# barathanaslan/whisper-ipa

Measured on AMD Instinct MI355X. Metric: audio-seconds/sec transcribed (whisper-small, 30s clips), higher is better.
Workload: dtype bf16

## Files before the change

### whisper_ipa_amd/csrc/cross_absorbed.hip

```cpp
#include <cstdlib>
#include <mutex>
#include <type_traits>

#include "attn_stream.h"
#include "wipa_common.h"

int wipa_cross_absorbed_loop_variant() {
    const char* e = getenv("WIPA_ABS_LOOP");
    const int v = e ? atoi(e) : 1;
    return (v >= 0 && v <= 3) ? v : 1;
}

namespace {

constexpr int FT = 32;
constexpr long long XA_RESIDENT_MB_SHARED = 16;
constexpr long long XA_RESIDENT_MB_LONE = -1;
typedef __attribute__((address_space(3))) void* lds_ptr_a;
typedef int v2i32 __attribute__((ext_vector_type(2)));

struct AbsParams {
    const __bf16* qp;
    const __bf16* xa;
    float* part_m;
    float* part_l;
    float* part_o;
    int Tk, n_splits, tiles_per_split, H;
    int resident_groups;
};

constexpr int POLICY_DEFAULT = 0, POLICY_NT = 2;

__device__ __forceinline__ int swz(int row) { return (row & 7) << 1; }

template <int D>
struct AbsCfg {
    static constexpr int NW = 4;
    static constexpr int ROWB = D * 2;
    static constexpr int TILE = FT * ROWB;
    static constexpr int SX = NW * 2 * 64 * 4 * (int)sizeof(float);
    static constexpr int NBUF = (3 * TILE + SX <= 160 * 1024) ? 3 : 2;
    static constexpr int SMEM = NBUF * TILE + SX;
};

template <int D>
__global__ __launch_bounds__(512, 1) void cross_absorbed_kernel(AbsParams p) {
    typedef AbsCfg<D> X;
    constexpr int NW = X::NW, ROWB = X::ROWB, TILE = X::TILE, NBUF = X::NBUF;
    constexpr int NDMA = TILE / 1024 / NW;
    constexpr int KS = D / NW / 32;
    constexpr int CT = D / NW / 16;
    static_assert(D % (32 * NW) == 0 && TILE % (1024 * NW) == 0, "width");
    extern __shared__ __attribute__((aligned(1024))) char smem[];
    float* sx = reinterpret_cast<float*>(smem + NBUF * TILE);
    const int tid = threadIdx.x, lane = tid & 63;
    const int wave = __builtin_amdgcn_readfirstlane(tid >> 6);
    const int l15 = lane & 15, g = lane >> 4;
    const int split = blockIdx.x, b = blockIdx.y;
    const int tile0 = split * p.tiles_per_split;
    const int n_tiles_total = (p.Tk + FT - 1) / FT;
    const int nt = max(0, min(p.tiles_per_split, n_tiles_total - tile0));
    const __bf16* xb = p.xa + (int64_t)b * p.Tk * D;

// ... 511 lines not shown

template <int D>
__global__ __launch_bounds__(64) void cross_absorb_q_kernel(const __bf16* __restrict__ q, int64_t q_rs, const __bf16* __restrict__ wkT,
                                                            __bf16* __restrict__ qp, int B, int H, float scale) {
    constexpr int CT = D / 4 / 16;
    const int lane = threadIdx.x & 63, wave = blockIdx.z;
    const int l15 = lane & 15, g = lane >> 4;
    const int h = blockIdx.x, b0 = blockIdx.y * 16;
    if (h >= H) {
        for (int e = lane; e < 16 * (D / 4); e += 64) {
            const int bb = b0 + e / (D / 4);
            if (bb < B) qp[((int64_t)bb * 16 + h) * D + wave * (D / 4) + e % (D / 4)] = (__bf16)0.f;
        }
        return;
    }
    const int bq = min(b0 + l15, B - 1);
    bf16x8 qa[2];
#pragma unroll
    for (int ks = 0; ks < 2; ++ks) qa[ks] = *reinterpret_cast<const bf16x8*>(q + (int64_t)bq * q_rs + h * 64 + 32 * ks + 8 * g);
    bf16x8 wb[CT][2];
#pragma unroll
    for (int i = 0; i < CT; ++i)
#pragma unroll
        for (int ks = 0; ks < 2; ++ks)
            wb[i][ks] = *reinterpret_cast<const bf16x8*>(wkT + (int64_t)(wave * (D / 4) + 16 * i + l15) * D + h * 64 + 32 * ks + 8 * g);
#pragma unroll
    for (int i = 0; i < CT; ++i) {
        const int c0 = wave * (D / 4) + 16 * i;
        f32x4 acc = f32x4{0.f, 0.f, 0.f, 0.f};
#pragma unroll
        for (int ks = 0; ks < 2; ++ks) acc = __builtin_amdgcn_mfma_f32_16x16x32_bf16(qa[ks], wb[i][ks], acc, 0, 0, 0);
#pragma unroll
        for (int r = 0; r < 4; ++r) {
            const int bb = b0 + 4 * g + r;
            if (bb < B) qp[((int64_t)bb * 16 + h) * D + c0 + l15] = (__bf16)(acc[r] * scale);
        }
    }
}

template <int D>
struct MergeCfg {
#ifndef WIPA_MERGE_KQ
#define WIPA_MERGE_KQ 96
#endif
#ifndef WIPA_MERGE_CL
#define WIPA_MERGE_CL 4
#endif
    static constexpr int KQ = (D % 96 == 0) ? WIPA_MERGE_KQ : (D == 512 ? 64 : 128);
    static constexpr int NWM = D / KQ;
    static constexpr int KS = KQ / 32;
    static constexpr int CL = WIPA_MERGE_CL;
};

template <int D, bool OUTP = false, int NS = 4>
__global__ __launch_bounds__(64 * MergeCfg<D>::NWM) void cross_merge_proj_kernel(
    const float* __restrict__ part_m, const float* __restrict__ part_l, const float* __restrict__ part_o, int n_splits,
    const __bf16* __restrict__ wv, const float* __restrict__ bv, __bf16* __restrict__ out, int64_t o_rs, int B,
    const __bf16* __restrict__ wo = nullptr, const float* __restrict__ bo = nullptr, float* __restrict__ slabs_out = nullptr,
    int64_t slab_stride = 0) {
    constexpr int KQ = MergeCfg<D>::KQ, KS = MergeCfg<D>::KS, NWM = MergeCfg<D>::NWM;
    static_assert(KQ % 32 == 0 && NWM * KQ == D, "width");
    constexpr int CL = MergeCfg<D>::CL;
    constexpr int NTO = D / 16;
    constexpr int NTOW = (NTO + NWM - 1) / NWM;
    __shared__ __attribute__((aligned(16))) float red[NWM][CL][64 + 4];
    __shared__ __attribute__((aligned(16))) __bf16 vh[OUTP ? CL : 1][64 + 8];
    const int tid = threadIdx.x, lane = tid & 63, w = tid >> 6;
    const int l15 = lane & 15, g = lane >> 4;
    const int h = blockIdx.x, b0 = blockIdx.y * CL;
    const int bc = min(b0 + (l15 & (CL - 1)), B - 1);
    bf16x8 wq[4][KS];
#pragma unroll
    for (int nt = 0; nt < 4; ++nt)
#pragma unroll
        for (int ks = 0; ks < KS; ++ks)
            wq[nt][ks] = *reinterpret_cast<const bf16x8*>(wv + (int64_t)(h * 64 + 16 * nt + l15) * D + w * KQ + 32 * ks + 8 * g);
    bf16x8 wof[OUTP ? NTOW : 1][2];
    if constexpr (OUTP) {
#pragma unroll
        for (int i = 0; i < NTOW; ++i) {
            const int nt = min(w * NTOW + i, NTO - 1);
#pragma unroll
            for (int ks = 0; ks < 2; ++ks)
                wof[i][ks] = *reinterpret_cast<const bf16x8*>(wo + (int64_t)(16 * nt + l15) * D + h * 64 + 32 * ks + 8 * g);
        }
    }
    float pm[NS], pl[NS];
#pragma unroll
    for (int s = 0; s < NS; ++s) {
        const int sc = NS == 4 ? min(s, n_splits - 1) : s;
        pm[s] = part_m[((int64_t)bc * n_splits + sc) * 16 + h];
        pl[s] = part_l[((int64_t)bc * n_splits + sc) * 16 + h];
    }
    f32x4 po[KS][NS][2];
#pragma unroll
    for (int ks = 0; ks < KS; ++ks)
#pragma unroll
        for (int s = 0; s < NS; ++s) {
            const int sc = NS == 4 ? min(s, n_splits - 1) : s;
            const float* pr = part_o + (((int64_t)bc * n_splits + sc) * 16 + h) * D + w * KQ + 32 * ks + 8 * g;
            po[ks][s][0] = *reinterpret_cast<const f32x4*>(pr);
            po[ks][s][1] = *reinterpret_cast<const f32x4*>(pr + 4);
        }
    __builtin_amdgcn_sched_barrier(0);
    float ws[NS];
    {
        float M = NEG_BIG;
#pragma unroll
        for (int s = 0; s < NS; ++s)
            if (NS < 4 || s < n_splits) M = fmaxf(M, pm[s]);
        float Lsum = 0.f;
#pragma unroll
        for (int s = 0; s < NS; ++s) {
            ws[s] = (NS < 4 || s < n_splits) ? __expf(pm[s] - M) : 0.f;
            Lsum = __builtin_fmaf(ws[s], pl[s], Lsum);
        }
        const float inv = 1.0f / Lsum;
#pragma unroll
        for (int s = 0; s < NS; ++s) ws[s] *= inv;
    }
    f32x4 acc[4] = {f32x4{0.f, 0.f, 0.f, 0.f}, f32x4{0.f, 0.f, 0.f, 0.f}, f32x4{0.f, 0.f, 0.f, 0.f}, f32x4{0.f, 0.f, 0.f, 0.f}};
#pragma unroll
    for (int ks = 0; ks < KS; ++ks) {
        f32x4 lo = {0.f, 0.f, 0.f, 0.f}, hi = {0.f, 0.f, 0.f, 0.f};
#pragma unroll
        for (int s = 0; s < NS; ++s) {
            const f32x4 w4 = {ws[s], ws[s], ws[s], ws[s]};
            lo = __builtin_elementwise_fma(w4, po[ks][s][0], lo);
            hi = __builtin_elementwise_fma(w4, po[ks][s][1], hi);
        }
        bf16x8 a;
#pragma unroll
        for (int e = 0; e < 4; ++e) {
            a[e] = (__bf16)lo[e];
            a[4 + e] = (__bf16)hi[e];
        }
#pragma unroll
        for (int nt = 0; nt < 4; ++nt) acc[nt] = __builtin_amdgcn_mfma_f32_16x16x32_bf16(a, wq[nt][ks], acc[nt], 0, 0, 0);
    }
    if (4 * g < CL) {
#pragma unroll
        for (int nt = 0; nt < 4; ++nt)
#pragma unroll
            for (int r = 0; r < 4; ++r)
                if (4 * g + r < CL) red[w][4 * g + r][16 * nt + l15] = acc[nt][r];
    }
    __syncthreads();
    for (int e = tid; e < CL * 64; e += 64 * NWM) {
        const int row = e >> 6, j = e & 63;
        float o = 0.f;
#pragma unroll
        for (int v = 0; v < NWM; ++v) o += red[v][row][j];
        const __bf16 val = (__bf16)(o + bv[h * 64 + j]);
        if constexpr (OUTP) vh[row][j] = val;
        else if (b0 + row < B) out[(int64_t)(b0 + row) * o_rs + h * 64 + j] = val;
    }
    if constexpr (OUTP) {
        __syncthreads();
        const bf16x8 a0 = *reinterpret_cast<const bf16x8*>(&vh[l15 & (CL - 1)][8 * g]);
        const bf16x8 a1 = *reinterpret_cast<const bf16x8*>(&vh[l15 & (CL - 1)][32 + 8 * g]);
#pragma unroll
        for (int i = 0; i < NTOW; ++i) {
            const int nt = w * NTOW + i;
            if (nt < NTO) {
                f32x4 acc2 = {0.f, 0.f, 0.f, 0.f};
                acc2 = __builtin_amdgcn_mfma_f32_16x16x32_bf16(a0, wof[i][0], acc2, 0, 0, 0);
                acc2 = __builtin_amdgcn_mfma_f32_16x16x32_bf16(a1, wof[i][1], acc2, 0, 0, 0);
                if (4 * g < CL) {
                    const float bias = (h == 0) ? bo[16 * nt + l15] : 0.f;
#pragma unroll
                    for (int r = 0; r < 4; ++r)
                        if (4 * g + r < CL && b0 + 4 * g + r < B)
                            slabs_out[(int64_t)h * slab_stride + (int64_t)(b0 + 4 * g + r) * D + 16 * nt + l15] = acc2[r] + bias;
                }
            }
        }
    }
}

struct AbsPrologueParams {
    const float* x_in;
    float* x_out;
    const float* slabs;
    const float* ln_w;
    const float* ln_b;
    const __bf16* wq;
    const float* bq;
    const __bf16* wkT;
    __bf16* qp;
    int64_t slab_stride;
    int n_slabs, B, H;
    float eps, q_scale, k_scale;
};

template <int D, int CG>
__global__ __launch_bounds__(512) void cross_absorb_prologue_kernel(AbsPrologueParams p) {
    constexpr int KS = D / 32;
    constexpr int KSW = (KS + 7) / 8;
    constexpr int NT = D / 16;
    constexpr int NTW = (NT + 7) / 8;
    constexpr int LROW = D + 8;
    constexpr int V4 = D / 256;
    static_assert(D % 256 == 0 || D == 384, "width");
    __shared__ __attribute__((aligned(16))) __bf16 lnx[16][LROW];
    __shared__ __attribute__((aligned(16))) float red[8][16][64 + 4];
    __shared__ __attribute__((aligned(16))) __bf16 qh[16][64 + 8];
    const int tid = threadIdx.x, lane = tid & 63;
    const int wave = __builtin_amdgcn_readfirstlane(tid >> 6);
// ... 70 lines not shown
            if (b0 + row < p.B) *reinterpret_cast<bf16x8*>(p.qp + ((int64_t)(b0 + row) * 16 + hp) * D + 8 * c8) = bf16x8{0, 0, 0, 0, 0, 0, 0, 0};
        }
    }
    __syncthreads();
    {
        f32x4 acc[4] = {f32x4{0.f, 0.f, 0.f, 0.f}, f32x4{0.f, 0.f, 0.f, 0.f}, f32x4{0.f, 0.f, 0.f, 0.f}, f32x4{0.f, 0.f, 0.f, 0.f}};
#pragma unroll
        for (int i = 0; i < KSW; ++i) {
            const int ks = wave * KSW + i;
            if (ks < KS) {
                const bf16x8 a = *reinterpret_cast<const bf16x8*>(&lnx[l15][32 * ks + 8 * g]);
#pragma unroll
                for (int nt = 0; nt < 4; ++nt) acc[nt] = __builtin_amdgcn_mfma_f32_16x16x32_bf16(a, wqf[nt][i], acc[nt], 0, 0, 0);
            }
        }
#pragma unroll
        for (int nt = 0; nt < 4; ++nt)
#pragma unroll
            for (int r = 0; r < 4; ++r) red[wave][4 * g + r][16 * nt + l15] = acc[nt][r];
    }
    __syncthreads();
#pragma unroll
    for (int i = 0; i < CG / 8; ++i) {
        const int e = tid + 512 * i, row = e >> 6, j = e & 63;
        float q = 0.f;
#pragma unroll
        for (int w = 0; w < 8; ++w) q += red[w][row][j];
        qh[row][j] = (__bf16)((q + p.bq[h * 64 + j]) * p.q_scale);
    }
    if constexpr (CG < 16) {
        for (int e = tid; e < (16 - CG) * 64; e += 512) qh[CG + (e >> 6)][e & 63] = (__bf16)0.f;
    }
    __syncthreads();
    {
        const bf16x8 a0 = *reinterpret_cast<const bf16x8*>(&qh[l15][8 * g]);
        const bf16x8 a1 = *reinterpret_cast<const bf16x8*>(&qh[l15][32 + 8 * g]);
#pragma unroll
        for (int i = 0; i < NTW; ++i) {
            const int nt = wave * NTW + i;
            if (nt < NT) {
                f32x4 acc = {0.f, 0.f, 0.f, 0.f};
                acc = __builtin_amdgcn_mfma_f32_16x16x32_bf16(a0, wkf[i][0], acc, 0, 0, 0);
                acc = __builtin_amdgcn_mfma_f32_16x16x32_bf16(a1, wkf[i][1], acc, 0, 0, 0);
#pragma unroll
                for (int r = 0; r < 4; ++r) {
                    const int bb_ = b0 + 4 * g + r;
                    if (4 * g + r < CG && bb_ < p.B) p.qp[((int64_t)bb_ * 16 + h) * D + 16 * nt + l15] = (__bf16)(acc[r] * p.k_scale);
                }
            }
        }
    }
}

template <int D, bool OUTP, typename... Args>
void launch_merge(int lv, int S, dim3 grid, hipStream_t s, Args... args) {
    constexpr int T = 64 * MergeCfg<D>::NWM;
    const int ns = (lv == 1 || lv == 3) ? S : 4;
    if (ns == 1) hipLaunchKernelGGL((cross_merge_proj_kernel<D, OUTP, 1>), grid, dim3(T), 0, s, args...);
    else if (ns == 2) hipLaunchKernelGGL((cross_merge_proj_kernel<D, OUTP, 2>), grid, dim3(T), 0, s, args...);
    else if (ns == 3) hipLaunchKernelGGL((cross_merge_proj_kernel<D, OUTP, 3>), grid, dim3(T), 0, s, args...);
    else hipLaunchKernelGGL((cross_merge_proj_kernel<D, OUTP, 4>), grid, dim3(T), 0, s, args...);
}

template <int D>
int launch_attn(int lv, const AbsParams& p_in, int B, hipStream_t s) {
    const char* e = getenv("WIPA_ABS_KERNEL");
    const bool pipe = lv == 1 || lv == 2;
    AbsParams p = p_in;
    p.resident_groups = wipa_cross_absorbed_resident_groups(B, D, p.Tk, p.n_splits);
    if ((e && atoi(e) == 1) || (D > 768 && !(e && atoi(e) == 2)))
        hipLaunchKernelGGL((cross_absorbed_kernel<D>), dim3(p.n_splits, B), dim3(64 * AbsCfg<D>::NW), AbsCfg<D>::SMEM, s, p);
    else if constexpr (D > 768) {
        if (pipe) hipLaunchKernelGGL((cross_absorbed_v2_kernel<D, 2, true>), dim3(p.n_splits, B), dim3(128), (AbsCfg2<D, 2>::SMEM), s, p);
        else hipLaunchKernelGGL((cross_absorbed_v2_kernel<D, 2, false>), dim3(p.n_splits, B), dim3(128), (AbsCfg2<D, 2>::SMEM), s, p);
    } else {
        static const int waves = [] { const char* w = getenv("WIPA_ABS_WAVES"); return w ? atoi(w) : 3; }();
        if (waves == 2 && pipe) hipLaunchKernelGGL((cross_absorbed_v2_kernel<D, 2, true>), dim3(p.n_splits, B), dim3(128), (AbsCfg2<D, 2>::SMEM), s, p);
        else if (waves == 2) hipLaunchKernelGGL((cross_absorbed_v2_kernel<D, 2, false>), dim3(p.n_splits, B), dim3(128), (AbsCfg2<D, 2>::SMEM), s, p);
        else if (pipe) hipLaunchKernelGGL((cross_absorbed_v2_kernel<D, 3, true>), dim3(p.n_splits, B), dim3(192), (AbsCfg2<D, 3>::SMEM), s, p);
        else hipLaunchKernelGGL((cross_absorbed_v2_kernel<D, 3, false>), dim3(p.n_splits, B), dim3(192), (AbsCfg2<D, 3>::SMEM), s, p);
    }
    return WIPA_OK;
}

AbsParams abs_params(void* scratch, int B, int d, int Tk, int S, int H, const void* xa) {
    char* sc = (char*)scratch;
    AbsParams p = {};
    p.qp = (const __bf16*)sc; p.xa = (const __bf16*)xa;
    p.part_m = (float*)(sc + (size_t)B * 16 * d * 2);
    p.part_l = p.part_m + (size_t)B * S * 16;
    p.part_o = p.part_l + (size_t)B * S * 16;
    p.Tk = Tk; p.n_splits = S; p.H = H;
    const int tiles = (Tk + FT - 1) / FT;
    p.tiles_per_split = (tiles + S - 1) / S;
    return p;
}

template <typename F>
int for_width(int d, F f) {
    if (d == 384) return f(std::integral_constant<int, 384>());
    if (d == 512) return f(std::integral_constant<int, 512>());
    if (d == 768) return f(std::integral_constant<int, 768>());
    if (d == 1024) return f(std::integral_constant<int, 1024>());
    return WIPA_ERR_ARG;
}

}

extern "C" int wipa_cross_absorbed_splits(int want, int Tk) {
    const int tiles = (Tk + FT - 1) / FT;
// ... 44 lines not shown
                                        hipFuncAttributeMaxDynamicSharedMemorySize, AbsCfg2<D, 3>::SMEM);
            if (e == hipSuccess)
                e = hipFuncSetAttribute(reinterpret_cast<const void*>(&cross_absorbed_v2_kernel<D, 3, false>),
                                        hipFuncAttributeMaxDynamicSharedMemorySize, AbsCfg2<D, 3>::SMEM);
        }
        if (e == hipSuccess)
            e = hipFuncSetAttribute(reinterpret_cast<const void*>(&cross_absorbed_v2_kernel<D, 2, true>),
                                    hipFuncAttributeMaxDynamicSharedMemorySize, AbsCfg2<D, 2>::SMEM);
        if (e == hipSuccess)
            e = hipFuncSetAttribute(reinterpret_cast<const void*>(&cross_absorbed_v2_kernel<D, 2, false>),
                                    hipFuncAttributeMaxDynamicSharedMemorySize, AbsCfg2<D, 2>::SMEM);
        return WIPA_OK;
    });
    WIPA_CHECK_HIP(e);
    done[wi] = true;
    return WIPA_OK;
}

extern "C" int wipa_cross_absorbed_stream(const void* xa, void* scratch, size_t scratch_bytes, int B, int H, int d, int Tk, int n_splits,
                                          wipa_stream_t stream) {
    WIPA_REQUIRE(xa && scratch && B > 0 && H >= 1 && H <= 16 && d == H * 64 && (d == 384 || d == 512 || d == 768 || d == 1024) && Tk >= 1 &&
                     n_splits >= 0 && n_splits <= 4,
                 "wipa_cross_absorbed_stream: bad arguments");
    WIPA_REQUIRE(scratch_bytes >= wipa_cross_absorbed_scratch_bytes(B, d, Tk), "wipa_cross_absorbed_stream: scratch too small");
    const int rc0 = wipa_cross_absorbed_init(d);
    if (rc0 != WIPA_OK) return rc0;
    const int S = wipa_cross_absorbed_splits(n_splits, Tk);
    const AbsParams p = abs_params(scratch, B, d, Tk, S, H, xa);
    const int rc = for_width(d, [&](auto width) { return launch_attn<decltype(width)::value>(wipa_cross_absorbed_loop_variant(), p, B, (hipStream_t)stream); });
    if (rc != WIPA_OK) return rc;
    WIPA_LAUNCH_CHECK();
    return WIPA_OK;
}

extern "C" int wipa_cross_absorbed_attention(const void* q, int64_t q_row_stride, const void* wkT, const void* xa, const void* wv,
                                             const float* bv, void* out, int64_t out_row_stride, void* scratch, size_t scratch_bytes,
                                             int B, int H, int d, int Tk, float k_scale, int n_splits, wipa_stream_t stream) {
    WIPA_REQUIRE(q && wkT && xa && wv && bv && out && scratch, "wipa_cross_absorbed_attention: null pointer");
    WIPA_REQUIRE(n_splits >= 0 && n_splits <= 4, "wipa_cross_absorbed_attention: n_splits %d (0 = default, 1..4)", n_splits);
    WIPA_REQUIRE(B > 0 && B <= 65535 && H >= 1 && H <= 16 && d == H * 64 && (d == 384 || d == 512 || d == 768 || d == 1024) && Tk >= 1,
                 "wipa_cross_absorbed_attention: bf16, <= 16 heads of 64, d in {384, 512, 768, 1024} (got H=%d d=%d)", H, d);
    WIPA_REQUIRE(q_row_stride % 8 == 0 && out_row_stride >= d && ((uintptr_t)q % 16) == 0 && ((uintptr_t)xa % 16) == 0 &&
                     ((uintptr_t)wkT % 16) == 0 && ((uintptr_t)wv % 16) == 0 && ((uintptr_t)scratch % 16) == 0,
                 "wipa_cross_absorbed_attention: operands must be 16-byte aligned");
    WIPA_REQUIRE((int64_t)Tk * d * 2 < ((int64_t)1 << 31), "wipa_cross_absorbed_attention: clip too long for 32-bit tile offsets");
    WIPA_REQUIRE(scratch_bytes >= wipa_cross_absorbed_scratch_bytes(B, d, Tk), "wipa_cross_absorbed_attention: scratch too small");
    hipStream_t s = (hipStream_t)stream;
    {
        const int rc0 = wipa_cross_absorbed_init(d);
        if (rc0 != WIPA_OK) return rc0;
    }
    const int S = wipa_cross_absorbed_splits(n_splits, Tk);
    const AbsParams p = abs_params(scratch, B, d, Tk, S, H, xa);
    const dim3 gq(16, (B + 15) / 16, 4), gm(H, (B + WIPA_MERGE_CL - 1) / WIPA_MERGE_CL);
    const int lv = wipa_cross_absorbed_loop_variant();
    const char* st_env = getenv("WIPA_ABS_STAGES");
    const int stages = st_env ? atoi(st_env) : 7;
    const int rc = for_width(d, [&](auto width) {
        constexpr int D = decltype(width)::value;
        int rc = WIPA_OK;
        if (stages & 1)
            hipLaunchKernelGGL((cross_absorb_q_kernel<D>), gq, dim3(64), 0, s, (const __bf16*)q, q_row_stride, (const __bf16*)wkT,
                               const_cast<__bf16*>(p.qp), B, H, k_scale);
        if (stages & 2) rc = launch_attn<D>(lv, p, B, s);
        if (rc == WIPA_OK && (stages & 4))
            launch_merge<D, false>(lv, S, gm, s, (const float*)p.part_m, (const float*)p.part_l, (const float*)p.part_o, S, (const __bf16*)wv, bv,
                                   (__bf16*)out, out_row_stride, B, (const __bf16*)nullptr, (const float*)nullptr, (float*)nullptr, (int64_t)0);
        return rc;
    });
    if (rc != WIPA_OK) return rc;
    WIPA_LAUNCH_CHECK();
    return WIPA_OK;
}

static int absorbed_block(const wipa_cross_block_desc* c, const void* wkT, const void* wv, const float* bv, const void* wo, const float* bo,
                          float* slabs_out, int64_t slab_stride, void* scratch, size_t scratch_bytes, wipa_stream_t stream);

extern "C" int wipa_decode_cross_absorbed_block(const wipa_cross_block_desc* c, const void* wkT, const void* wv, const float* bv, void* scratch,
                                                size_t scratch_bytes, wipa_stream_t stream) {
    WIPA_REQUIRE(c && c->out, "wipa_decode_cross_absorbed_block: null pointer");
    return absorbed_block(c, wkT, wv, bv, nullptr, nullptr, nullptr, 0, scratch, scratch_bytes, stream);
}

extern "C" int wipa_decode_cross_absorbed_block_out(const wipa_cross_block_desc* c, const void* wkT, const void* wv, const float* bv,
                                                    const void* wo, const float* bo, float* slabs_out, int64_t slab_stride, void* scratch,
                                                    size_t scratch_bytes, wipa_stream_t stream) {
    WIPA_REQUIRE(c && wo && bo && slabs_out && slab_stride >= (int64_t)c->B * c->d && ((uintptr_t)wo % 16) == 0,
                 "wipa_decode_cross_absorbed_block_out: null pointer / short slab stride");
    return absorbed_block(c, wkT, wv, bv, wo, bo, slabs_out, slab_stride, scratch, scratch_bytes, stream);
}

static int absorbed_block(const wipa_cross_block_desc* c, const void* wkT, const void* wv, const float* bv, const void* wo, const float* bo,
                          float* slabs_out, int64_t slab_stride, void* scratch, size_t scratch_bytes, wipa_stream_t stream) {
    WIPA_REQUIRE(c && c->x_in && c->x_out && c->ln_w && c->ln_b && c->wq && c->bq && c->kv && (c->out || wo) && wkT && wv && bv && scratch,
                 "wipa_decode_cross_absorbed_block: null pointer");
    WIPA_REQUIRE(c->x_in != c->x_out, "wipa_decode_cross_absorbed_block: x_out must not alias x_in");
    const int B = c->B, H = c->H, d = c->d, Tk = c->Tk;
    WIPA_REQUIRE(c->dtype == WIPA_BF16 && B > 0 && B <= 65535 * 16 && H >= 1 && H <= 16 && d == H * 64 &&
                     (d == 384 || d == 512 || d == 768 || d == 1024) && Tk >= 1 && c->n_slabs >= 0 && c->n_slabs <= 4 && !c->bias_o &&
                     c->cross_splits >= 0 && c->cross_splits <= 4,
                 "wipa_decode_cross_absorbed_block: bf16, <= 16 heads of 64, d in {384, 512, 768, 1024}, <= 4 slabs, no separate bias, "
                 "cross_splits 0..4");
    WIPA_REQUIRE(c->n_slabs == 0 || c->slabs, "wipa_decode_cross_absorbed_block: slabs missing");
    WIPA_REQUIRE((int64_t)Tk * d * 2 < ((int64_t)1 << 31), "wipa_decode_cross_absorbed_block: clip too long for 32-bit tile offsets");
    WIPA_REQUIRE(scratch_bytes >= wipa_cross_absorbed_scratch_bytes(B, d, Tk), "wipa_decode_cross_absorbed_block: scratch too small");
    hipStream_t s = (hipStream_t)stream;
    const int S = wipa_cross_absorbed_splits(c->cross_splits, Tk);
    const AbsParams p = abs_params(scratch, B, d, Tk, S, H, c->kv);
    AbsPrologueParams q = {};
    q.x_in = c->x_in; q.x_out = c->x_out; q.slabs = c->slabs; q.ln_w = c->ln_w; q.ln_b = c->ln_b;
    q.wq = (const __bf16*)c->wq; q.bq = c->bq; q.wkT = (const __bf16*)wkT; q.qp = const_cast<__bf16*>(p.qp);
    q.slab_stride = c->slab_stride; q.n_slabs = c->n_slabs; q.B = B; q.H = H;
    q.eps = c->eps; q.q_scale = c->qk_scale; q.k_scale = c->qk_scale;
    const int lv = wipa_cross_absorbed_loop_variant();
    static const int cg = [] { const char* e = getenv("WIPA_ABS_PROLOGUE_CLIPS"); return e ? atoi(e) : 8; }();
    const dim3 gp(H, cg == 8 ? (B + 7) / 8 : (B + 15) / 16), gm(H, (B + WIPA_MERGE_CL - 1) / WIPA_MERGE_CL);
    const int rc = for_width(d, [&](auto width) {
        constexpr int D = decltype(width)::value;
        if (cg == 8) hipLaunchKernelGGL((cross_absorb_prologue_kernel<D, 8>), gp, dim3(512), 0, s, q);
        else hipLaunchKernelGGL((cross_absorb_prologue_kernel<D, 16>), gp, dim3(512), 0, s, q);
        const int rc = launch_attn<D>(lv, p, B, s);
        if (rc == WIPA_OK && wo)
            launch_merge<D, true>(lv, S, gm, s, (const float*)p.part_m, (const float*)p.part_l, (const float*)p.part_o, S, (const __bf16*)wv, bv,
                                  (__bf16*)nullptr, (int64_t)d, B, (const __bf16*)wo, bo, slabs_out, slab_stride);
        else if (rc == WIPA_OK)
            launch_merge<D, false>(lv, S, gm, s, (const float*)p.part_m, (const float*)p.part_l, (const float*)p.part_o, S, (const __bf16*)wv, bv,
                                   (__bf16*)c->out, (int64_t)d, B, (const __bf16*)nullptr, (const float*)nullptr, (float*)nullptr, (int64_t)0);
        return rc;
    });
    if (rc != WIPA_OK) return rc;
    WIPA_LAUNCH_CHECK();
    return WIPA_OK;
}
```

### whisper_ipa_amd/csrc/runtime.hip

```cpp
#include <algorithm>
#include <cstdarg>
#include <cstdlib>
#include <cstring>
#include <strings.h>
#include <map>
#include <mutex>
#include <tuple>
#include <vector>

#include "wipa_common.h"

static thread_local char g_err[512] = "";
void wipa_set_error(const char* fmt, ...) {
    va_list ap;
    va_start(ap, fmt);
    vsnprintf(g_err, sizeof(g_err), fmt, ap);
    va_end(ap);
}
extern "C" const char* wipa_last_error(void) { return g_err; }
extern "C" int wipa_version(void) { return 100; }

extern "C" int wipa_stream_create_cu_limited(int n_cus, wipa_stream_t* out) {
    int dev = 0, total = 0;
    WIPA_CHECK_HIP(hipGetDevice(&dev));
// ... 832 lines not shown
    hipStream_t s = (hipStream_t)stream;
    char* st = (char*)state;
    const DecScratch S = dec_scratch(cfg, B);
    RT_CALL(wipa_decode_fused_init());
    RT_CALL(wipa_gemm_init());
    WIPA_CHECK_HIP(hipMemsetAsync(st + L.tokens, 0, (size_t)B * L.ld_tok * 4, s));
    WIPA_CHECK_HIP(hipMemsetAsync(st + L.pos, 0, 512, s));
    WIPA_CHECK_HIP(hipMemsetAsync(st + L.sum_logprobs, 0, (size_t)B * 4, s));
    WIPA_CHECK_HIP(hipMemsetAsync(st + L.scratch + S.posd, 0, 8, s));
    int t4[4] = {0, 0, 0, 0};
    for (int i = 0; i < n_init; ++i) t4[i] = initial_tokens_host[i];
    hipLaunchKernelGGL(fill_tokens_kernel, dim3((B + 63) / 64), dim3(64), 0, s, (int32_t*)(st + L.tokens), L.ld_tok, B, n_init,
                       t4[0], t4[1], t4[2], t4[3], (const int32_t*)nullptr);
    WIPA_LAUNCH_CHECK();
    return WIPA_OK;
}

extern "C" int wipa_decoder_run(const wipa_model_cfg* cfg, const void* const* w, void* state, size_t state_bytes, int B, int n_init,
                                int eot, const float* mask_first, const float* mask_always, int n_steps, int use_graph,
                                wipa_stream_t stream) {
    return wipa_decoder_run_rules(cfg, w, state, state_bytes, B, n_init, eot, mask_first, mask_always, n_steps, use_graph, nullptr, stream);
}

extern "C" int wipa_decoder_run_rules(const wipa_model_cfg* cfg, const void* const* w, void* state, size_t state_bytes, int B, int n_init,
                                      int eot, const float* mask_first, const float* mask_always, int n_steps, int use_graph,
                                      const wipa_decode_rules* rules, wipa_stream_t stream) {
    RT_CALL(cfg_check(cfg));
    SplitScope split_scope(cfg);
    WIPA_REQUIRE(w && state && mask_first && mask_always && B > 0 && n_steps >= 0, "wipa_decoder_run: bad arguments");
    RT_CALL(rules_servable("wipa_decoder_run_rules", cfg, B, eot, rules));
    RulesScope rules_scope(rules);
    W8Scope w8_scope(cfg, w);
    const wipa_dec_layout L = dec_layout(cfg, B);
    RT_CALL(state_fits("wipa_decoder_run", L, state_bytes));
    char* st = (char*)state;
    hipStream_t s = (hipStream_t)stream;
    RT_CALL(init_before_capture(cfg));
    if (n_steps == 0) return WIPA_OK;
    WIPA_CHECK_HIP(hipMemsetAsync(done_counter_of(st, L), 0, sizeof(int32_t), s));
    if (step_needs_head(cfg, B)) RT_CALL(enqueue_step_head(cfg, w, st, L, B, stream));
    const bool lean_ok = !use_fused_step(cfg, B) && logits_fused(cfg, B);
    struct LeanScope {
        explicit LeanScope(bool v) { t_lean_logits = v; }
        ~LeanScope() { t_lean_logits = false; }
    };
    if (!use_graph || !graphs_allowed()) {
        for (int i = 0; i < n_steps; ++i) {
            LeanScope lean(lean_ok && i + 1 < n_steps);
            RT_CALL(enqueue_decode_step(cfg, w, st, L, B, n_init, eot, mask_first, mask_always, stream));
        }
        return WIPA_OK;
    }
    WIPA_REQUIRE(s != nullptr, "wipa_decoder_run: graph capture needs a non-default stream");
    const int variant = cfg->dtype * 2 + t_f32_split + 4 * decode_mode(cfg, B) + 16 * cfg->dec_w_dtype + 64 * cfg->dec_cross_absorbed * (absorbed_block_fused() ? 2 : 1) + 256 * (int)tail_fused() + 512 * (int)absorbed_merge_out() + 1024 * cfg->dec_cross_splits + 8192 * (int)lean_ok + 16384 * (cfg->dec_cross_absorbed ? wipa_cross_absorbed_loop_variant() : 0);
    auto step_graph = [&](bool lean, hipGraphExec_t* out) -> int {
        hipGraphExec_t exec = nullptr;
        const GraphKey key(state, (const void*)w, (const void*)mask_first, (const void*)mask_always, B, n_init, eot, variant, cfg->weights_generation,
                           lean ? 2 : 0, rules ? rules->timestamp_begin : 0, rules ? rules->no_timestamps : 0,
                           rules ? rules->max_initial_timestamp_index : 0);
        {
            std::lock_guard<std::mutex> lk(g_graph_mu);
            auto it = g_graphs.find(key);
            if (it != g_graphs.end()) exec = it->second;
        }
        if (!exec) {
            hipGraph_t graph = nullptr;
            WIPA_CHECK_HIP(hipStreamBeginCapture(s, hipStreamCaptureModeRelaxed));
            int rc;
            {
                LeanScope scope(lean);
                rc = enqueue_decode_step(cfg, w, st, L, B, n_init, eot, mask_first, mask_always, stream);
            }
            const hipError_t ee = hipStreamEndCapture(s, &graph);
            if (rc != WIPA_OK) {
                if (graph) hipGraphDestroy(graph);
                return rc;
            }
            WIPA_CHECK_HIP(ee);
            WIPA_CHECK_HIP(hipGraphInstantiate(&exec, graph, nullptr, nullptr, 0));
            WIPA_CHECK_HIP(hipGraphDestroy(graph));
            std::lock_guard<std::mutex> lk(g_graph_mu);
            g_graphs[key] = exec;
        }
        *out = exec;
        return WIPA_OK;
    };
    hipGraphExec_t full = nullptr, lean = nullptr;
    RT_CALL(step_graph(false, &full));
    if (lean_ok && n_steps > 1) RT_CALL(step_graph(true, &lean));
    for (int i = 0; i < n_steps; ++i) WIPA_CHECK_HIP(hipGraphLaunch((lean && i + 1 < n_steps) ? lean : full, s));
    return WIPA_OK;
}

extern "C" int wipa_decoder_prefill(const wipa_model_cfg* cfg, const void* const* w, void* state, size_t state_bytes, int B,
                                    int n_init, int eot, const float* mask_first, const float* mask_always, int use_graph,
                                    wipa_stream_t stream) {
    return wipa_decoder_prefill_rules(cfg, w, state, state_bytes, B, n_init, eot, mask_first, mask_always, use_graph, nullptr, stream);
}

extern "C" int wipa_decoder_prefill_rules(const wipa_model_cfg* cfg, const void* const* w, void* state, size_t state_bytes, int B,
                                          int n_init, int eot, const float* mask_first, const float* mask_always, int use_graph,
                                          const wipa_decode_rules* rules, wipa_stream_t stream) {
    RT_CALL(cfg_check(cfg));
    SplitScope split_scope(cfg);
    WIPA_REQUIRE(w && state && mask_first && mask_always && B > 0, "wipa_decoder_prefill: bad arguments");
    RT_CALL(rules_servable("wipa_decoder_prefill_rules", cfg, B, eot, rules));
    RulesScope rules_scope(rules);
    WIPA_REQUIRE(n_init >= 1 && n_init <= MAX_PROMPT, "wipa_decoder_prefill: 1..%d prompt tokens (got %d)", MAX_PROMPT, n_init);
    W8Scope w8_scope(cfg, w);
    const wipa_dec_layout L = dec_layout(cfg, B);
    RT_CALL(state_fits("wipa_decoder_prefill", L, state_bytes));
    char* st = (char*)state;
    auto enqueue = [&]() -> int {
        if (n_init == 1) {
            if (step_needs_head(cfg, B)) RT_CALL(enqueue_step_head(cfg, w, st, L, B, stream));
            return enqueue_decode_step(cfg, w, st, L, B, n_init, eot, mask_first, mask_always, stream);
        }
        return enqueue_prefill(cfg, w, st, L, B, n_init, eot, mask_first, mask_always, stream);
    };
    hipStream_t s = (hipStream_t)stream;
    RT_CALL(init_before_capture(cfg));
    WIPA_CHECK_HIP(hipMemsetAsync(done_counter_of(st, L), 0, sizeof(int32_t), s));
    if (!use_graph || s == nullptr || !graphs_allowed()) return enqueue();
    hipGraphExec_t exec = nullptr;
    const GraphKey key(state, (const void*)w, (const void*)mask_first, (const void*)mask_always, B, n_init, eot, cfg->dtype * 2 + t_f32_split + 4 * decode_mode(cfg, B) + 16 * cfg->dec_w_dtype + 64 * cfg->dec_cross_absorbed * (absorbed_block_fused() ? 2 : 1) + 256 * (int)tail_fused() + 512 * (int)absorbed_merge_out() + 1024 * cfg->dec_cross_splits + 8192 * (int)(!use_fused_step(cfg, B) && logits_fused(cfg, B)) + 16384 * (cfg->dec_cross_absorbed ? wipa_cross_absorbed_loop_variant() : 0), cfg->weights_generation, 1,
                       rules ? rules->timestamp_begin : 0, rules ? rules->no_timestamps : 0, rules ? rules->max_initial_timestamp_index : 0);
    {
        std::lock_guard<std::mutex> lk(g_graph_mu);
        auto it = g_graphs.find(key);
        if (it != g_graphs.end()) exec = it->second;
    }
    if (!exec) {
        hipGraph_t graph = nullptr;
        WIPA_CHECK_HIP(hipStreamBeginCapture(s, hipStreamCaptureModeRelaxed));
        const int rc = enqueue();
        const hipError_t ee = hipStreamEndCapture(s, &graph);
        if (rc != WIPA_OK) {
            if (graph) hipGraphDestroy(graph);
            return rc;
        }
        WIPA_CHECK_HIP(ee);
        WIPA_CHECK_HIP(hipGraphInstantiate(&exec, graph, nullptr, nullptr, 0));
        WIPA_CHECK_HIP(hipGraphDestroy(graph));
        std::lock_guard<std::mutex> lk(g_graph_mu);
        g_graphs[key] = exec;
    }
    WIPA_CHECK_HIP(hipGraphLaunch(exec, s));
    return WIPA_OK;
}

extern "C" int wipa_decoder_release(void* state) {
    std::lock_guard<std::mutex> lk(g_graph_mu);
    for (auto it = g_graphs.begin(); it != g_graphs.end();) {
        if (std::get<0>(it->first) == state) {
            hipGraphExecDestroy(it->second);
            it = g_graphs.erase(it);
        } else {
            ++it;
        }
    }
    return WIPA_OK;
}

namespace {
struct TfWs {
    size_t x, ln, qkv, q, ao, h, ckv, total;
};
TfWs tf_ws(const wipa_model_cfg* c, int B, int T) {
    const size_t e = wipa_dtype_size(c->dtype), d = c->n_text_state, M = (size_t)B * T;
    TfWs w;
    size_t o = 0;
    w.x = o;   o += align256(M * d * 4);
    w.ln = o;  o += align256(M * d * e);
    w.qkv = o; o += align256(M * 3 * d * e);
    w.q = o;   o += align256(M * d * e);
    w.ao = o;  o += align256(M * d * e);
    w.h = o;   o += align256(M * 4 * d * e);
    w.ckv = o; o += align256((size_t)B * 2 * c->n_text_head * c->n_audio_ctx * 64 * e);
// ... 89 lines not shown
```

### whisper_ipa_amd/csrc/wipa_common.h

```cpp
#pragma once
#include <hip/hip_runtime.h>
#include <stdint.h>
#include <stdio.h>

#include "wipa.h"

typedef __attribute__((ext_vector_type(8))) __bf16 bf16x8;
typedef __attribute__((ext_vector_type(4))) __bf16 bf16x4;
typedef __attribute__((ext_vector_type(4))) float f32x4;
typedef __attribute__((ext_vector_type(16))) float f32x16;

#define WIPA_WAVE 64

void wipa_set_error(const char* fmt, ...);
int wipa_decode_fused_init();
int wipa_gemm_init();
int wipa_cross_absorbed_loop_variant();

#define WIPA_CHECK_HIP(expr)                                                        \
    do {                                                                            \
        hipError_t _e = (expr);                                                     \
        if (_e != hipSuccess) {                                                     \
            wipa_set_error("%s:%d %s -> %s", __FILE__, __LINE__, #expr, hipGetErrorString(_e)); \
            return WIPA_ERR_HIP;                                                    \
        }                                                                           \
    } while (0)

#define WIPA_REQUIRE(cond, ...)                \
    do {                                       \
        if (!(cond)) {                         \
            wipa_set_error(__VA_ARGS__);       \
            return WIPA_ERR_ARG;               \
        }                                      \
    } while (0)

#define WIPA_LAUNCH_CHECK()                                                          \
    do {                                                                             \
        hipError_t _e = hipGetLastError();                                           \
        if (_e != hipSuccess) {                                                      \
            wipa_set_error("%s:%d launch -> %s", __FILE__, __LINE__, hipGetErrorString(_e)); \
            return WIPA_ERR_HIP;                                                     \
        }                                                                            \
    } while (0)

static inline size_t wipa_dtype_size(int dt) { return dt == WIPA_BF16 ? 2 : 4; }

#ifdef __HIPCC__
__device__ __forceinline__ float wipa_bf16_to_f32(unsigned short h) {
    return __uint_as_float(((unsigned int)h) << 16);
}

template <typename T>
__device__ __forceinline__ float to_f32(T v);
template <>
__device__ __forceinline__ float to_f32<float>(float v) { return v; }
template <>
__device__ __forceinline__ float to_f32<__bf16>(__bf16 v) { return (float)v; }

template <typename T>
__device__ __forceinline__ T from_f32(float v);
template <>
__device__ __forceinline__ float from_f32<float>(float v) { return v; }
template <>
__device__ __forceinline__ __bf16 from_f32<__bf16>(float v) { return (__bf16)v; }

template <typename T>
struct Vec16;
template <>
struct Vec16<float> {
    static constexpr int EPL = 4;
// ... 93 lines not shown
```

Baseline: 27720.

## Split cross-attention merge projection over output column halves with 8-clip tiles

For D=768 without the fused out-projection, the merge+V-projection kernel gets a new grid shape. It now uses 8 clips per workgroup and splits the head's 64 output columns across two workgroups along z, with each workgroup computing 32 columns. This is used only when the resulting grid has at most 256 workgroups, and it is on by default behind WIPA_STEP_PLACEMENT. The goal is to spread the small decode-step merge across more CUs and cut per-workgroup MFMA and weight-register work. The cost is that each split re-reads the partial attention outputs and recomputes the softmax merge weights.

```diff
diff --git a/whisper_ipa_amd/csrc/cross_absorbed.hip b/whisper_ipa_amd/csrc/cross_absorbed.hip
--- a/whisper_ipa_amd/csrc/cross_absorbed.hip
+++ b/whisper_ipa_amd/csrc/cross_absorbed.hip
@@ -9,6 +9,11 @@
     const char* e = getenv("WIPA_ABS_LOOP");
     const int v = e ? atoi(e) : 1;
     return (v >= 0 && v <= 3) ? v : 1;
+}
+
+int wipa_step_placement() {
+    const char* e = getenv("WIPA_STEP_PLACE");
+    return (e && atoi(e) == 0) ? 0 : 1;
 }
 
 namespace {
@@ -626,7 +631,7 @@
     static constexpr int CL = WIPA_MERGE_CL;
 };
 
-template <int D, bool OUTP = false, int NS = 4>
+template <int D, bool OUTP = false, int NS = 4, int CL = MergeCfg<D>::CL, int CT = 4>
 __global__ __launch_bounds__(64 * MergeCfg<D>::NWM) void cross_merge_proj_kernel(
     const float* __restrict__ part_m, const float* __restrict__ part_l, const float* __restrict__ part_o, int n_splits,
     const __bf16* __restrict__ wv, const float* __restrict__ bv, __bf16* __restrict__ out, int64_t o_rs, int B,
@@ -634,21 +639,22 @@
     int64_t slab_stride = 0) {
     constexpr int KQ = MergeCfg<D>::KQ, KS = MergeCfg<D>::KS, NWM = MergeCfg<D>::NWM;
     static_assert(KQ % 32 == 0 && NWM * KQ == D, "width");
-    constexpr int CL = MergeCfg<D>::CL;
+    static_assert((CT == 4 || !OUTP) && (CT == 1 || CT == 2 || CT == 4), "the out projection needs the head's 64 values in one workgroup");
     constexpr int NTO = D / 16;
     constexpr int NTOW = (NTO + NWM - 1) / NWM;
-    __shared__ __attribute__((aligned(16))) float red[NWM][CL][64 + 4];
+    __shared__ __attribute__((aligned(16))) float red[NWM][CL][16 * CT + 4];
     __shared__ __attribute__((aligned(16))) __bf16 vh[OUTP ? CL : 1][64 + 8];
     const int tid = threadIdx.x, lane = tid & 63, w = tid >> 6;
     const int l15 = lane & 15, g = lane >> 4;
     const int h = blockIdx.x, b0 = blockIdx.y * CL;
+    const int c0 = CT < 4 ? 16 * CT * (int)blockIdx.z : 0;
     const int bc = min(b0 + (l15 & (CL - 1)), B - 1);
-    bf16x8 wq[4][KS];
-#pragma unroll
-    for (int nt = 0; nt < 4; ++nt)
+    bf16x8 wq[CT][KS];
+#pragma unroll
+    for (int nt = 0; nt < CT; ++nt)
 #pragma unroll
         for (int ks = 0; ks < KS; ++ks)
-            wq[nt][ks] = *reinterpret_cast<const bf16x8*>(wv + (int64_t)(h * 64 + 16 * nt + l15) * D + w * KQ + 32 * ks + 8 * g);
+            wq[nt][ks] = *reinterpret_cast<const bf16x8*>(wv + (int64_t)(h * 64 + c0 + 16 * nt + l15) * D + w * KQ + 32 * ks + 8 * g);
     bf16x8 wof[OUTP ? NTOW : 1][2];
     if constexpr (OUTP) {
 #pragma unroll
@@ -693,7 +699,9 @@
 #pragma unroll
         for (int s = 0; s < NS; ++s) ws[s] *= inv;
     }
-    f32x4 acc[4] = {f32x4{0.f, 0.f, 0.f, 0.f}, f32x4{0.f, 0.f, 0.f, 0.f}, f32x4{0.f, 0.f, 0.f, 0.f}, f32x4{0.f, 0.f, 0.f, 0.f}};
+    f32x4 acc[CT];
+#pragma unroll
+    for (int nt = 0; nt < CT; ++nt) acc[nt] = f32x4{0.f, 0.f, 0.f, 0.f};
 #pragma unroll
     for (int ks = 0; ks < KS; ++ks) {
         f32x4 lo = {0.f, 0.f, 0.f, 0.f}, hi = {0.f, 0.f, 0.f, 0.f};
@@ -710,24 +718,24 @@
             a[4 + e] = (__bf16)hi[e];
         }
 #pragma unroll
-        for (int nt = 0; nt < 4; ++nt) acc[nt] = __builtin_amdgcn_mfma_f32_16x16x32_bf16(a, wq[nt][ks], acc[nt], 0, 0, 0);
+        for (int nt = 0; nt < CT; ++nt) acc[nt] = __builtin_amdgcn_mfma_f32_16x16x32_bf16(a, wq[nt][ks], acc[nt], 0, 0, 0);
     }
     if (4 * g < CL) {
 #pragma unroll
-        for (int nt = 0; nt < 4; ++nt)
+        for (int nt = 0; nt < CT; ++nt)
 #pragma unroll
             for (int r = 0; r < 4; ++r)
                 if (4 * g + r < CL) red[w][4 * g + r][16 * nt + l15] = acc[nt][r];
     }
     __syncthreads();
-    for (int e = tid; e < CL * 64; e += 64 * NWM) {
-        const int row = e >> 6, j = e & 63;
+    for (int e = tid; e < CL * 16 * CT; e += 64 * NWM) {
+        const int row = e / (16 * CT), j = e % (16 * CT);
         float o = 0.f;
 #pragma unroll
         for (int v = 0; v < NWM; ++v) o += red[v][row][j];
-        const __bf16 val = (__bf16)(o + bv[h * 64 + j]);
+        const __bf16 val = (__bf16)(o + bv[h * 64 + c0 + j]);
         if constexpr (OUTP) vh[row][j] = val;
-        else if (b0 + row < B) out[(int64_t)(b0 + row) * o_rs + h * 64 + j] = val;
+        else if (b0 + row < B) out[(int64_t)(b0 + row) * o_rs + h * 64 + c0 + j] = val;
     }
     if constexpr (OUTP) {
         __syncthreads();
@@ -904,10 +912,23 @@
     }
 }
 
+constexpr int PLACE_MAX_WORKGROUPS = 256;
+
 template <int D, bool OUTP, typename... Args>
-void launch_merge(int lv, int S, dim3 grid, hipStream_t s, Args... args) {
+void launch_merge(int lv, int S, bool place, int H, int B, hipStream_t s, Args... args) {
     constexpr int T = 64 * MergeCfg<D>::NWM;
     const int ns = (lv == 1 || lv == 3) ? S : 4;
+    if constexpr (D == 768 && !OUTP) {
+        const dim3 g2(H, (B + 7) / 8, 2);
+        if (place && (int64_t)g2.x * g2.y * g2.z <= PLACE_MAX_WORKGROUPS) {
+            if (ns == 1) hipLaunchKernelGGL((cross_merge_proj_kernel<D, false, 1, 8, 2>), g2, dim3(T), 0, s, args...);
+            else if (ns == 2) hipLaunchKernelGGL((cross_merge_proj_kernel<D, false, 2, 8, 2>), g2, dim3(T), 0, s, args...);
+            else if (ns == 3) hipLaunchKernelGGL((cross_merge_proj_kernel<D, false, 3, 8, 2>), g2, dim3(T), 0, s, args...);
+            else hipLaunchKernelGGL((cross_merge_proj_kernel<D, false, 4, 8, 2>), g2, dim3(T), 0, s, args...);
+            return;
+        }
+    }
+    const dim3 grid(H, (B + WIPA_MERGE_CL - 1) / WIPA_MERGE_CL);
     if (ns == 1) hipLaunchKernelGGL((cross_merge_proj_kernel<D, OUTP, 1>), grid, dim3(T), 0, s, args...);
     else if (ns == 2) hipLaunchKernelGGL((cross_merge_proj_kernel<D, OUTP, 2>), grid, dim3(T), 0, s, args...);
     else if (ns == 3) hipLaunchKernelGGL((cross_merge_proj_kernel<D, OUTP, 3>), grid, dim3(T), 0, s, args...);
@@ -1058,8 +1079,9 @@
     }
     const int S = wipa_cross_absorbed_splits(n_splits, Tk);
     const AbsParams p = abs_params(scratch, B, d, Tk, S, H, xa);
-    const dim3 gq(16, (B + 15) / 16, 4), gm(H, (B + WIPA_MERGE_CL - 1) / WIPA_MERGE_CL);
+    const dim3 gq(16, (B + 15) / 16, 4);
     const int lv = wipa_cross_absorbed_loop_variant();
+    const bool place_merge = wipa_step_placement() != 0;
     const char* st_env = getenv("WIPA_ABS_STAGES");
     const int stages = st_env ? atoi(st_env) : 7;
     const int rc = for_width(d, [&](auto width) {
@@ -1070,7 +1092,7 @@
                                const_cast<__bf16*>(p.qp), B, H, k_scale);
         if (stages & 2) rc = launch_attn<D>(lv, p, B, s);
         if (rc == WIPA_OK && (stages & 4))
-            launch_merge<D, false>(lv, S, gm, s, (const float*)p.part_m, (const float*)p.part_l, (const float*)p.part_o, S, (const __bf16*)wv, bv,
+            launch_merge<D, false>(lv, S, place_merge, H, B, s, (const float*)p.part_m, (const float*)p.part_l, (const float*)p.part_o, S, (const __bf16*)wv, bv,
                                    (__bf16*)out, out_row_stride, B, (const __bf16*)nullptr, (const float*)nullptr, (float*)nullptr, (int64_t)0);
         return rc;
     });
@@ -1120,17 +1142,18 @@
     q.eps = c->eps; q.q_scale = c->qk_scale; q.k_scale = c->qk_scale;
     const int lv = wipa_cross_absorbed_loop_variant();
     static const int cg = [] { const char* e = getenv("WIPA_ABS_PROLOGUE_CLIPS"); return e ? atoi(e) : 8; }();
-    const dim3 gp(H, cg == 8 ? (B + 7) / 8 : (B + 15) / 16), gm(H, (B + WIPA_MERGE_CL - 1) / WIPA_MERGE_CL);
+    const dim3 gp(H, cg == 8 ? (B + 7) / 8 : (B + 15) / 16);
+    const bool place_merge = wipa_step_placement() != 0;
     const int rc = for_width(d, [&](auto width) {
         constexpr int D = decltype(width)::value;
         if (cg == 8) hipLaunchKernelGGL((cross_absorb_prologue_kernel<D, 8>), gp, dim3(512), 0, s, q);
         else hipLaunchKernelGGL((cross_absorb_prologue_kernel<D, 16>), gp, dim3(512), 0, s, q);
         const int rc = launch_attn<D>(lv, p, B, s);
         if (rc == WIPA_OK && wo)
-            launch_merge<D, true>(lv, S, gm, s, (const float*)p.part_m, (const float*)p.part_l, (const float*)p.part_o, S, (const __bf16*)wv, bv,
+            launch_merge<D, true>(lv, S, false, H, B, s, (const float*)p.part_m, (const float*)p.part_l, (const float*)p.part_o, S, (const __bf16*)wv, bv,
                                   (__bf16*)nullptr, (int64_t)d, B, (const __bf16*)wo, bo, slabs_out, slab_stride);
         else if (rc == WIPA_OK)
-            launch_merge<D, false>(lv, S, gm, s, (const float*)p.part_m, (const float*)p.part_l, (const float*)p.part_o, S, (const __bf16*)wv, bv,
+            launch_merge<D, false>(lv, S, place_merge, H, B, s, (const float*)p.part_m, (const float*)p.part_l, (const float*)p.part_o, S, (const __bf16*)wv, bv,
                                    (__bf16*)c->out, (int64_t)d, B, (const __bf16*)nullptr, (const float*)nullptr, (float*)nullptr, (int64_t)0);
         return rc;
     });
diff --git a/whisper_ipa_amd/csrc/runtime.hip b/whisper_ipa_amd/csrc/runtime.hip
--- a/whisper_ipa_amd/csrc/runtime.hip
+++ b/whisper_ipa_amd/csrc/runtime.hip
@@ -908,7 +908,7 @@
         return WIPA_OK;
     }
     WIPA_REQUIRE(s != nullptr, "wipa_decoder_run: graph capture needs a non-default stream");
-    const int variant = cfg->dtype * 2 + t_f32_split + 4 * decode_mode(cfg, B) + 16 * cfg->dec_w_dtype + 64 * cfg->dec_cross_absorbed * (absorbed_block_fused() ? 2 : 1) + 256 * (int)tail_fused() + 512 * (int)absorbed_merge_out() + 1024 * cfg->dec_cross_splits + 8192 * (int)lean_ok + 16384 * (cfg->dec_cross_absorbed ? wipa_cross_absorbed_loop_variant() : 0);
+    const int variant = cfg->dtype * 2 + t_f32_split + 4 * decode_mode(cfg, B) + 16 * cfg->dec_w_dtype + 64 * cfg->dec_cross_absorbed * (absorbed_block_fused() ? 2 : 1) + 256 * (int)tail_fused() + 512 * (int)absorbed_merge_out() + 1024 * cfg->dec_cross_splits + 8192 * (int)lean_ok + 16384 * (cfg->dec_cross_absorbed ? wipa_cross_absorbed_loop_variant() : 0) + 65536 * (cfg->dec_cross_absorbed ? wipa_step_placement() : 0);
     auto step_graph = [&](bool lean, hipGraphExec_t* out) -> int {
         hipGraphExec_t exec = nullptr;
         const GraphKey key(state, (const void*)w, (const void*)mask_first, (const void*)mask_always, B, n_init, eot, variant, cfg->weights_generation,
@@ -979,7 +979,7 @@
     WIPA_CHECK_HIP(hipMemsetAsync(done_counter_of(st, L), 0, sizeof(int32_t), s));
     if (!use_graph || s == nullptr || !graphs_allowed()) return enqueue();
     hipGraphExec_t exec = nullptr;
-    const GraphKey key(state, (const void*)w, (const void*)mask_first, (const void*)mask_always, B, n_init, eot, cfg->dtype * 2 + t_f32_split + 4 * decode_mode(cfg, B) + 16 * cfg->dec_w_dtype + 64 * cfg->dec_cross_absorbed * (absorbed_block_fused() ? 2 : 1) + 256 * (int)tail_fused() + 512 * (int)absorbed_merge_out() + 1024 * cfg->dec_cross_splits + 8192 * (int)(!use_fused_step(cfg, B) && logits_fused(cfg, B)) + 16384 * (cfg->dec_cross_absorbed ? wipa_cross_absorbed_loop_variant() : 0), cfg->weights_generation, 1,
+    const GraphKey key(state, (const void*)w, (const void*)mask_first, (const void*)mask_always, B, n_init, eot, cfg->dtype * 2 + t_f32_split + 4 * decode_mode(cfg, B) + 16 * cfg->dec_w_dtype + 64 * cfg->dec_cross_absorbed * (absorbed_block_fused() ? 2 : 1) + 256 * (int)tail_fused() + 512 * (int)absorbed_merge_out() + 1024 * cfg->dec_cross_splits + 8192 * (int)(!use_fused_step(cfg, B) && logits_fused(cfg, B)) + 16384 * (cfg->dec_cross_absorbed ? wipa_cross_absorbed_loop_variant() : 0) + 65536 * (cfg->dec_cross_absorbed ? wipa_step_placement() : 0), cfg->weights_generation, 1,
                        rules ? rules->timestamp_begin : 0, rules ? rules->no_timestamps : 0, rules ? rules->max_initial_timestamp_index : 0);
     {
         std::lock_guard<std::mutex> lk(g_graph_mu);
diff --git a/whisper_ipa_amd/csrc/wipa_common.h b/whisper_ipa_amd/csrc/wipa_common.h
--- a/whisper_ipa_amd/csrc/wipa_common.h
+++ b/whisper_ipa_amd/csrc/wipa_common.h
@@ -16,6 +16,7 @@
 int wipa_decode_fused_init();
 int wipa_gemm_init();
 int wipa_cross_absorbed_loop_variant();
+int wipa_step_placement();
 
 #define WIPA_CHECK_HIP(expr)                                                        \
     do {                                                                            \
```

After: 27810, median of 6. No clear change (+0.4%).
